# autonomousvision/LaRa

Hardware: AMD Instinct MI355X
Metric: novel-view frames/sec @512x512 (4-view in, 2DGS fwd+bwd) (higher is better)
Workload: dtype f32 raster + bf16-MFMA/f32-accumulate encoder (+ bf16-autocast coarse decoder MLP, as the reference's bf16-mixed)

## Files before the change

lara_amd/csrc/finedec.hip:

```cpp
#include "common.h"
#include "wave.h"
#include "../../include/lara_finedec.h"

namespace {

constexpr int FD = 80, NH = 8, CD = 8, NV = 4, HID = 64, SH = 12, TQ = NH * CD;

__device__ __forceinline__ int crow(const int tile, const int r, const int hf) { return tile * 32 + (r >> 2) * 8 + hf * 4 + (r & 3); }
__device__ __forceinline__ f32x16 mfma2(const float a, const float b, const f32x16 c) {
    return __builtin_amdgcn_mfma_f32_32x32x2f32(a, b, c, 0, 0, 0);
}
#define FD_FENCE(i, every) do { if (((i) % (every)) == (every) - 1) asm volatile("" ::: "memory"); } while (0)

__device__ __forceinline__ f32x16 zero16() {
    f32x16 z;
#pragma unroll
    for (int i = 0; i < 16; i++) z[i] = 0.f;
    return z;
}

constexpr int L_WQKT = 0;
constexpr int L_W1T = L_WQKT + FD * TQ;
constexpr int L_W2T = L_W1T + TQ * HID;
constexpr int L_B1 = L_W2T + HID * 32;
// ... 232 lines not shown
#pragma unroll
                for (int c = 0; c < 4; c++) {
                    dt[c] += dsc * pf[j][c];
                    dpf[j][c] += p[h][j] * du[mt][r0 + c] + dsc * t[mt][r0 + c];
                }
            }
#pragma unroll
            for (int c = 0; c < 4; c++) du[mt][r0 + c] = dt[c];
            asm volatile("" ::: "memory");
        }
        if (live) {
            store64(DT_g, pt, du);
#pragma unroll
            for (int j = 0; j < NV; j++)
#pragma unroll
                for (int c = 0; c < 4; c++) dpf_g[(int64_t)(j * CD + hf * 4 + c) * n + pt] = dpf[j][c];
        }
#pragma unroll
        for (int ft = 0; ft < 3; ft++) {
            f32x16 dx = zero16();
#pragma unroll
            for (int mt = 0; mt < 2; mt++)
#pragma unroll
                for (int r = 0; r < 16; r++) {
                    dx = mfma2(sw[L_WQK + crow(mt, r, hf) * 96 + ft * 32 + col], du[mt][r], dx);
                    FD_FENCE(r, 8);
                }
            if (live) {
#pragma unroll
                for (int q = 0; q < 4; q++) {
                    const int f0 = ft * 32 + q * 8 + hf * 4;
                    if (f0 < FD) *(float4 *)(dxn_g + pt * FD + f0) = make_float4(dx[4 * q], dx[4 * q + 1], dx[4 * q + 2], dx[4 * q + 3]);
                }
            }
        }
    }
}


__global__ void __launch_bounds__(256)
fine_ln_fwd_kernel(const int n, const float *__restrict__ x_g, const float *__restrict__ gamma, const float *__restrict__ beta,
                   const float eps, float *__restrict__ xn_g, float2 *__restrict__ stats) {
    __shared__ float sg[FD], sb[FD];
    if (threadIdx.x < FD) { sg[threadIdx.x] = gamma[threadIdx.x]; sb[threadIdx.x] = beta[threadIdx.x]; }
    __syncthreads();
    const int64_t i = (int64_t)blockIdx.x * 256 + threadIdx.x;
    if (i >= n) return;
    const float4 *x4 = (const float4 *)(x_g + i * FD);
    float4 v[FD / 4];
    float sum = 0.f;
#pragma unroll
    for (int k = 0; k < FD / 4; k++) { v[k] = x4[k]; sum += (v[k].x + v[k].y) + (v[k].z + v[k].w); }
    const float mean = sum * (1.0f / FD);
    float var = 0.f;
#pragma unroll
    for (int k = 0; k < FD / 4; k++) {
        const float a = v[k].x - mean, b = v[k].y - mean, c = v[k].z - mean, d = v[k].w - mean;
        var += (a * a + b * b) + (c * c + d * d);
    }
    const float rstd = 1.0f / sqrtf(var * (1.0f / FD) + eps);
    float4 *o4 = (float4 *)(xn_g + i * FD);
#pragma unroll
    for (int k = 0; k < FD / 4; k++) {
        float4 o;
        o.x = (v[k].x - mean) * rstd * sg[4 * k] + sb[4 * k];
        o.y = (v[k].y - mean) * rstd * sg[4 * k + 1] + sb[4 * k + 1];
        o.z = (v[k].z - mean) * rstd * sg[4 * k + 2] + sb[4 * k + 2];
        o.w = (v[k].w - mean) * rstd * sg[4 * k + 3] + sb[4 * k + 3];
        o4[k] = o;
    }
    stats[i] = make_float2(mean, rstd);
}

__device__ __forceinline__ float wave_sum_to_lane63(float x) {
    x += dpp_move<0xB1, 0xf>(x);
    x += dpp_move<0x4E, 0xf>(x);
    x += dpp_move<0x141, 0xf>(x);
    x += dpp_move<0x140, 0xf>(x);
    x += dpp_move<0x142, 0xa>(x);
    x += dpp_move<0x143, 0xc>(x);
    return x;
}

__global__ void __launch_bounds__(256)
fine_ln_bwd_kernel(const int n, const float *__restrict__ x_g, const float *__restrict__ gamma, const float2 *__restrict__ stats,
                   const float *__restrict__ dxn_g, float *__restrict__ dx_g, float *__restrict__ partials) {
    __shared__ float sg[FD];
    __shared__ float part[4][2 * FD];
    if (threadIdx.x < FD) sg[threadIdx.x] = gamma[threadIdx.x];
    __syncthreads();
    const int64_t i = (int64_t)blockIdx.x * 256 + threadIdx.x;
    const bool on = i < n;
    const int lane = threadIdx.x & 63, wave = threadIdx.x >> 6;
    float4 xh[FD / 4], g[FD / 4];
    float2 st = make_float2(0.f, 0.f);
    if (on) st = stats[i];
    float s1 = 0.f, s2 = 0.f;
#pragma unroll
    for (int k = 0; k < FD / 4; k++) {
        float4 xv = make_float4(0.f, 0.f, 0.f, 0.f), dv = xv;
        if (on) { xv = ((const float4 *)(x_g + i * FD))[k]; dv = ((const float4 *)(dxn_g + i * FD))[k]; }
        xh[k] = make_float4((xv.x - st.x) * st.y, (xv.y - st.x) * st.y, (xv.z - st.x) * st.y, (xv.w - st.x) * st.y);
        const float pg[4] = {dv.x * xh[k].x, dv.y * xh[k].y, dv.z * xh[k].z, dv.w * xh[k].w};
        const float pb[4] = {dv.x, dv.y, dv.z, dv.w};
#pragma unroll
        for (int q = 0; q < 4; q++) {
            const float a = wave_sum_to_lane63(pg[q]), b = wave_sum_to_lane63(pb[q]);
            if (lane == 63) { part[wave][4 * k + q] = a; part[wave][FD + 4 * k + q] = b; }
        }
        g[k] = make_float4(dv.x * sg[4 * k], dv.y * sg[4 * k + 1], dv.z * sg[4 * k + 2], dv.w * sg[4 * k + 3]);
        s1 += (g[k].x + g[k].y) + (g[k].z + g[k].w);
        s2 += (g[k].x * xh[k].x + g[k].y * xh[k].y) + (g[k].z * xh[k].z + g[k].w * xh[k].w);
    }
    if (on) {
        const float m1 = s1 * (1.0f / FD), m2 = s2 * (1.0f / FD);
        float4 *o4 = (float4 *)(dx_g + i * FD);
#pragma unroll
        for (int k = 0; k < FD / 4; k++)
            o4[k] = make_float4(st.y * (g[k].x - m1 - xh[k].x * m2), st.y * (g[k].y - m1 - xh[k].y * m2),
                                st.y * (g[k].z - m1 - xh[k].z * m2), st.y * (g[k].w - m1 - xh[k].w * m2));
    }
    __syncthreads();
    if (threadIdx.x < 2 * FD)
        partials[(size_t)blockIdx.x * 2 * FD + threadIdx.x] =
            ((part[0][threadIdx.x] + part[1][threadIdx.x]) + part[2][threadIdx.x]) + part[3][threadIdx.x];
}

constexpr int FW_SLAB = 512;
constexpr int FW_OUT = 64 * 80 + 64 * 64 + 64 + 12 * 64 + 12;
constexpr int FW_O_W1 = 64 * 80, FW_O_B1 = FW_O_W1 + 64 * 64, FW_O_W2 = FW_O_B1 + 64, FW_O_B2 = FW_O_W2 + 12 * 64;

template <int AV, int BV>
__device__ __forceinline__ void fw_store(float *__restrict__ out, const int ldo, const int i_rows, const int j_cols, const int lane,
                                         const f32x16 (&acc)[AV][BV]) {
    const int cB = lane & 31, kh = lane >> 5;
#pragma unroll
    for (int ea = 0; ea < AV; ea++)
#pragma unroll
        for (int eb = 0; eb < BV; eb++)
#pragma unroll
            for (int e = 0; e < 16; e++) {
                const int i = AV * ((e & 3) + 8 * (e >> 2) + 4 * kh) + ea, j = BV * cB + eb;
                if (i < i_rows && j < j_cols) out[(size_t)i * ldo + j] = acc[ea][eb][e];
            }
}

__global__ void __launch_bounds__(192)
fine_wgrad_kernel(const int n, const float *__restrict__ xn, const float *__restrict__ U, const float *__restrict__ HID_,
                  const float *__restrict__ DH, const float *__restrict__ DT, const float *__restrict__ d_sh,
                  float *__restrict__ part) {
    const int wave = threadIdx.x >> 6, lane = threadIdx.x & 63;
    const int row0 = blockIdx.x * FW_SLAB, rows = min(FW_SLAB, n - row0);
    float *out = part + (size_t)blockIdx.x * FW_OUT;
    const int kk = lane >> 5, c = lane & 31;
    constexpr int UN = 8;
    if (wave < 2) {
        f32x16 acc[2][2];
#pragma unroll
        for (int a = 0; a < 2; a++)
#pragma unroll
            for (int b = 0; b < 2; b++)
#pragma unroll
                for (int e = 0; e < 16; e++) acc[a][b][e] = 0.f;
        const bool b_ok = c < FD / 4;
        for (int r = 0; r < rows; r += 2 * UN) {
            float2 av[UN], bv[UN];
#pragma unroll
            for (int u = 0; u < UN; u++) {
                const int rr = r + 2 * u + kk;
                const bool in = rr < rows;
                av[u] = in ? *(const float2 *)(DT + (size_t)(row0 + rr) * 64 + 2 * c) : make_float2(0.f, 0.f);
                bv[u] = (in && b_ok) ? *(const float2 *)(xn + (size_t)(row0 + rr) * FD + 4 * c + 2 * wave) : make_float2(0.f, 0.f);
            }
#pragma unroll
            for (int u = 0; u < UN; u++) {
                acc[0][0] = mfma2(av[u].x, bv[u].x, acc[0][0]);
                acc[0][1] = mfma2(av[u].x, bv[u].y, acc[0][1]);
                acc[1][0] = mfma2(av[u].y, bv[u].x, acc[1][0]);
                acc[1][1] = mfma2(av[u].y, bv[u].y, acc[1][1]);
            }
        }
        const int kh = lane >> 5;
#pragma unroll
        for (int ea = 0; ea < 2; ea++)
#pragma unroll
            for (int eb = 0; eb < 2; eb++)
#pragma unroll
                for (int e = 0; e < 16; e++) {
                    const int i = 2 * ((e & 3) + 8 * (e >> 2) + 4 * kh) + ea, j = 4 * c + 2 * wave + eb;
                    if (j < FD) out[(size_t)i * FD + j] = acc[ea][eb][e];
                }
    } else {
        f32x16 acc1[2][2], acc2[1][2];
#pragma unroll
        for (int b = 0; b < 2; b++)
#pragma unroll
            for (int e = 0; e < 16; e++) { acc1[0][b][e] = 0.f; acc1[1][b][e] = 0.f; acc2[0][b][e] = 0.f; }
        float cs1x = 0.f, cs1y = 0.f, cs2 = 0.f;
        const bool s_ok = c < SH;
        for (int r = 0; r < rows; r += 2 * UN) {
            float2 dh[UN], uu[UN], hh[UN];
            float ds[UN];
#pragma unroll
// ... 133 lines not shown
```

lara_amd/csrc/pointfeat.hip:

```cpp
#include "common.h"
#include "../../include/lara_pointfeat.h"

namespace {

constexpr int PF_MAX_VIEWS = 8;

struct PfP {
    int n, V, h, w;
    const float *points, *w2cs, *ixts, *img_ref, *image, *acc, *depth;
    int vtot;
};

__device__ __forceinline__ size_t map_pixel(const PfP &p, const size_t i) {
    if (p.vtot == 0) return i;
    const size_t hw = (size_t)p.h * p.w, v = i / hw, pix = i - v * hw, y = pix / p.w, x = pix - y * p.w;
    return (y * p.vtot + v) * p.w + x;
}

struct Tap {
    int idx[4];
    float wgt[4];
    float wx, wy;
    bool in[4];
};
// ... 98 lines not shown
        const Proj pr = project(p, v, px, py, pz);
        const Tap t = taps(pr.x, pr.y, p.h, p.w);
        float val[4][8];
#pragma unroll
        for (int k = 0; k < 4; k++) {
            if (t.in[k]) chan8(packed, hw, v, t.idx[k], val[k]);
            else
#pragma unroll
                for (int c = 0; c < 8; c++) val[k][c] = 0.f;
        }
        float gx = 0.f, gy = 0.f, gz = 0.f, gc[8];
#pragma unroll
        for (int c = 0; c < 8; c++) {
            float g = g_out[((size_t)v * 8 + c) * p.n + i];
            if (c == 7) {
                const float s = t.wgt[0] * val[0][c] + t.wgt[1] * val[1][c] + t.wgt[2] * val[2][c] + t.wgt[3] * val[3][c];
                const float d = s - pr.z, sg = d > 0.f ? 1.f : d < 0.f ? -1.f : 0.f;
                gz -= sg * g;
                g *= sg;
            }
            gc[c] = g;
            gx += g * ((val[1][c] - val[0][c]) * (1.f - t.wy) + (val[3][c] - val[2][c]) * t.wy);
            gy += g * ((val[2][c] - val[0][c]) * (1.f - t.wx) + (val[3][c] - val[1][c]) * t.wx);
        }
        if (dpacked) {
#pragma unroll
            for (int k = 0; k < 4; k++) {
                s_off[wave][lane][k] = t.in[k] ? (int)(((size_t)v * hw + t.idx[k]) * 8) : -1;
                s_wgt[wave][lane][k] = t.wgt[k];
            }
#pragma unroll
            for (int c = 0; c < 8; c++) s_g[wave][lane][c] = gc[c];
        }
        const float inv = 1.0f / pr.z;
        const float dqx = gx * inv, dqy = gy * inv, dqz = gz - (gx * pr.x + gy * pr.y) * inv;
        const float *m = p.w2cs + v * 16, *k = p.ixts + v * 9;
        const float dcx = k[0] * dqx + k[3] * dqy + k[6] * dqz, dcy = k[1] * dqx + k[4] * dqy + k[7] * dqz,
                    dcz = k[2] * dqx + k[5] * dqy + k[8] * dqz;
        dpx = m[0] * dcx + m[4] * dcy + m[8] * dcz;
        dpy = m[1] * dcx + m[5] * dcy + m[9] * dcz;
        dpz = m[2] * dcx + m[6] * dcy + m[10] * dcz;
    }
    if (dpacked) {
        __builtin_amdgcn_wave_barrier();
        const int ch = lane & 7;
#pragma unroll 4
        for (int r = 0; r < 32; r++) {
            const int item = r * 8 + (lane >> 3), th = item >> 2, k = item & 3;
            const int off = s_off[wave][th][k];
            if (off >= 0 && ch >= 3) atomicAdd(dpacked + off + ch, s_wgt[wave][th][k] * s_g[wave][th][ch]);
        }
    }
#pragma unroll
    for (int o = 1; o < VP; o <<= 1) {
        dpx += __shfl_xor(dpx, o, 64); dpy += __shfl_xor(dpy, o, 64); dpz += __shfl_xor(dpz, o, 64);
    }
    if (active && v == 0) {
        d_points[3 * (size_t)i] = dpx; d_points[3 * (size_t)i + 1] = dpy; d_points[3 * (size_t)i + 2] = dpz;
    }
}

template <int VP>
int launch_fwd(const PfP &p, const float4 *packed, float *out, hipStream_t s) {
    const size_t threads = (size_t)p.n * VP;
    L2D_LAUNCH_IN_SCOPE(s, (point_feats_fwd_kernel<VP>), dim3((unsigned)((threads + 255) / 256)), dim3(256), 0, p, packed, out);
    return LARA2DGS_OK;
}
template <int VP>
int launch_bwd(const PfP &p, const float4 *packed, const float *g_out, float *d_points, float *dpacked, hipStream_t s) {
    const size_t threads = (size_t)p.n * VP;
    L2D_LAUNCH_IN_SCOPE(s, (point_feats_bwd_kernel<VP>), dim3((unsigned)((threads + 255) / 256)), dim3(256), 0, p, packed, g_out,
                        d_points, dpacked);
    return LARA2DGS_OK;
}
int launch_pack(const PfP &p, float4 *packed, hipStream_t s) {
    const size_t n = (size_t)p.V * p.h * p.w;
    L2D_LAUNCH_IN_SCOPE(s, pack_stack_kernel, dim3((unsigned)((n + 255) / 256)), dim3(256), 0, p, packed);
    return LARA2DGS_OK;
}

struct RowsP {
    const float *src[LARA_ROWS_MAX];
    float *dst[LARA_ROWS_MAX];
    int width[LARA_ROWS_MAX], first[LARA_ROWS_MAX + 1];
    const int64_t *idx;
    int n, count;
};
template <bool SCATTER>
__global__ void __launch_bounds__(256) take_rows_kernel(const RowsP p) {
    const int total = p.first[p.count];
    const int t = blockIdx.x * 256 + threadIdx.x;
    if (t >= p.n * total) return;
    const int r = t / total, c = t - r * total;
    int k = 0;
    while (k + 1 < p.count && c >= p.first[k + 1]) k++;
    const int w = p.width[k], cc = c - p.first[k];
    const size_t far = (size_t)p.idx[r] * w + cc, near = (size_t)r * w + cc;
    if (SCATTER) p.dst[k][far] = p.src[k][near];
    else p.dst[k][near] = p.src[k][far];
}

__global__ void __launch_bounds__(256) voxel_rows_fwd_kernel(const int n, const int c4, const long long *__restrict__ vox,
                                                            const float4 *__restrict__ x, float4 *__restrict__ out) {
    const long long t = (long long)blockIdx.x * 256 + threadIdx.x;
    if (t >= (long long)n * c4) return;
    const int r = (int)(t / c4), c = (int)(t - (long long)r * c4);
    out[t] = x[(size_t)vox[r] * c4 + c];
}
__global__ void __launch_bounds__(256) voxel_rows_bwd_kernel(const int n, const int c4, const long long *__restrict__ vox,
                                                            const float4 *__restrict__ g, float4 *__restrict__ dx) {
    const long long t = (long long)blockIdx.x * 256 + threadIdx.x;
    if (t >= (long long)n * c4) return;
    const int r = (int)(t / c4), c = (int)(t - (long long)r * c4);
    const long long v = vox[r];
    if (r > 0 && vox[r - 1] == v) return;
    float4 a = g[t];
    for (int q = r + 1; q < n && vox[q] == v; q++) {
        const float4 b = g[(size_t)q * c4 + c];
        a.x += b.x; a.y += b.y; a.z += b.z; a.w += b.w;
    }
    dx[(size_t)v * c4 + c] = a;
}

}

extern "C" {

int lara_voxel_rows(int32_t n, int32_t width, const int64_t *vox, const float *src, float *dst, int32_t backward, void *stream) {
    if (n < 0 || width <= 0 || (width & 3)) return LARA2DGS_E_INVALID;
    if (n == 0) return LARA2DGS_OK;
    if (!vox || !src || !dst) return LARA2DGS_E_INVALID;
    hipStream_t s = (hipStream_t)stream;
    const int c4 = width / 4;
    const unsigned blocks = (unsigned)(((long long)n * c4 + 255) / 256);
    {
        L2D_PROF(backward ? "voxel_rows_bwd" : "voxel_rows_fwd", s);
        if (backward) L2D_LAUNCH_IN_SCOPE(s, voxel_rows_bwd_kernel, dim3(blocks), dim3(256), 0, n, c4, (const long long *)vox, (const float4 *)src, (float4 *)dst);
        else L2D_LAUNCH_IN_SCOPE(s, voxel_rows_fwd_kernel, dim3(blocks), dim3(256), 0, n, c4, (const long long *)vox, (const float4 *)src, (float4 *)dst);
    }
    return LARA2DGS_OK;
}

int64_t lara_point_feats_workspace_bytes(int32_t V, int32_t h, int32_t w) {
    if (V <= 0 || V > PF_MAX_VIEWS || h <= 0 || w <= 0 || (int64_t)V * h * w * 8 >= (1ll << 31)) return LARA2DGS_E_INVALID;
    return (int64_t)V * h * w * 32 * 2;
}

int lara_point_feats_forward(int32_t n, int32_t V, int32_t h, int32_t w, const float *points, const float *w2cs,
                             const float *ixts, const float *img_ref, const float *image, const float *acc_map,
                             const float *depth, float *out, void *workspace, void *stream) {
    return lara_point_feats_forward_concat(n, V, 0, h, w, points, w2cs, ixts, img_ref, image, acc_map, depth, out, workspace, stream);
}

int lara_point_feats_forward_concat(int32_t n, int32_t V, int32_t row_views, int32_t h, int32_t w, const float *points,
                                    const float *w2cs, const float *ixts, const float *img_ref, const float *image,
                                    const float *acc_map, const float *depth, float *out, void *workspace, void *stream) {
    if (row_views < 0 || (row_views > 0 && row_views < V)) return LARA2DGS_E_INVALID;
    if (n < 0 || V <= 0 || V > PF_MAX_VIEWS || h <= 0 || w <= 0 || (int64_t)V * h * w * 8 >= (1ll << 31)) return LARA2DGS_E_INVALID;
    if (n == 0) return LARA2DGS_OK;
    if (!points || !w2cs || !ixts || !img_ref || !image || !acc_map || !depth || !out || !workspace) return LARA2DGS_E_INVALID;
    hipStream_t s = (hipStream_t)stream;
    const PfP p{n, V, h, w, points, w2cs, ixts, img_ref, image, acc_map, depth, row_views};
    float4 *packed = (float4 *)workspace;
    {
        L2D_PROF("point_feats_pack", s);
        L2D_TRY(launch_pack(p, packed, s));
    }
    {
        L2D_PROF("point_feats_fwd", s);
        if (V == 1) L2D_TRY(launch_fwd<1>(p, packed, out, s));
        else if (V == 2) L2D_TRY(launch_fwd<2>(p, packed, out, s));
        else if (V <= 4) L2D_TRY(launch_fwd<4>(p, packed, out, s));
        else L2D_TRY(launch_fwd<8>(p, packed, out, s));
    }
    return LARA2DGS_OK;
}

int lara_point_feats_backward(int32_t n, int32_t V, int32_t h, int32_t w, const float *points, const float *w2cs,
                              const float *ixts, const float *img_ref, const float *image, const float *acc_map,
                              const float *depth, const float *g_out, float *d_points, float *d_image,
                              float *d_acc_map, float *d_depth, void *workspace, void *stream) {
    return lara_point_feats_backward_concat(n, V, 0, h, w, points, w2cs, ixts, img_ref, image, acc_map, depth, g_out, d_points,
                                            d_image, d_acc_map, d_depth, workspace, stream);
}

int lara_point_feats_backward_concat(int32_t n, int32_t V, int32_t row_views, int32_t h, int32_t w, const float *points,
                                     const float *w2cs, const float *ixts, const float *img_ref, const float *image,
                                     const float *acc_map, const float *depth, const float *g_out, float *d_points,
                                     float *d_image, float *d_acc_map, float *d_depth, void *workspace, void *stream) {
    if (row_views < 0 || (row_views > 0 && row_views < V)) return LARA2DGS_E_INVALID;
    if (n < 0 || V <= 0 || V > PF_MAX_VIEWS || h <= 0 || w <= 0 || (int64_t)V * h * w * 8 >= (1ll << 31)) return LARA2DGS_E_INVALID;
    if (n == 0) return LARA2DGS_OK;
    if (!points || !w2cs || !ixts || !img_ref || !image || !acc_map || !depth || !g_out || !d_points || !workspace)
        return LARA2DGS_E_INVALID;
    hipStream_t s = (hipStream_t)stream;
    const PfP p{n, V, h, w, points, w2cs, ixts, img_ref, image, acc_map, depth, row_views};
    const size_t npix = (size_t)V * h * w;
    float4 *packed = (float4 *)workspace;
    const bool maps = d_image || d_acc_map || d_depth;
    float *dpacked = maps ? (float *)workspace + npix * 8 : nullptr;
    {
        L2D_PROF("point_feats_pack", s);
        L2D_TRY(launch_pack(p, packed, s));
        if (maps) L2D_HIP(hipMemsetAsync(dpacked, 0, npix * 32, s));
    }
    {
        L2D_PROF("point_feats_bwd", s);
        if (V == 1) L2D_TRY(launch_bwd<1>(p, packed, g_out, d_points, dpacked, s));
        else if (V == 2) L2D_TRY(launch_bwd<2>(p, packed, g_out, d_points, dpacked, s));
        else if (V <= 4) L2D_TRY(launch_bwd<4>(p, packed, g_out, d_points, dpacked, s));
        else L2D_TRY(launch_bwd<8>(p, packed, g_out, d_points, dpacked, s));
        if (maps)
            L2D_LAUNCH_IN_SCOPE(s, unpack_grad_kernel, dim3((unsigned)((npix + 255) / 256)), dim3(256), 0, p, (const float4 *)dpacked, npix,
                                d_image, d_acc_map, d_depth);
    }
    return LARA2DGS_OK;
}


int lara_take_rows(int32_t n, const int64_t *idx, int32_t count, const lara_rows_item *items, int32_t scatter, void *stream) {
    if (n < 0 || count < 0 || count > LARA_ROWS_MAX) return LARA2DGS_E_INVALID;
    if (n == 0 || count == 0) return LARA2DGS_OK;
    if (!idx || !items) return LARA2DGS_E_INVALID;
    RowsP p{};
    p.n = n; p.count = count; p.idx = idx;
    int total = 0;
    for (int k = 0; k < count; k++) {
        if (!items[k].src || !items[k].dst || items[k].width <= 0) return LARA2DGS_E_INVALID;
        p.src[k] = items[k].src; p.dst[k] = items[k].dst; p.width[k] = items[k].width; p.first[k] = total;
        total += items[k].width;
    }
    p.first[count] = total;
    if ((int64_t)n * total >= (1ll << 31)) return LARA2DGS_E_INVALID;
    hipStream_t s = (hipStream_t)stream;
    const unsigned blocks = (unsigned)(((int64_t)n * total + 255) / 256);
    {
        L2D_PROF(scatter ? "take_rows_bwd" : "take_rows_fwd", s);
        if (scatter) L2D_LAUNCH_IN_SCOPE(s, take_rows_kernel<true>, dim3(blocks), dim3(256), 0, p);
        else L2D_LAUNCH_IN_SCOPE(s, take_rows_kernel<false>, dim3(blocks), dim3(256), 0, p);
    }
    return LARA2DGS_OK;
}

}
```

lara_amd/csrc/preprocess.hip:

```cpp
#include "common.h"
#include "tilebox.h"

static_assert(TILE == 16, "tilebox.h's l2d_tight_rect cuts to 16-pixel tiles");

namespace {

__device__ __constant__ float kSH_C2[5] = {1.0925484305920792f, -1.0925484305920792f,
                                           0.31539156525252005f, -1.0925484305920792f,
                                           0.5462742152960396f};
__device__ __constant__ float kSH_C3[7] = {-0.5900435899266435f, 2.890611442640554f,
                                           -0.4570457994644658f, 0.3731763325901154f,
                                           -0.4570457994644658f, 1.445305721320277f,
                                           -0.5900435899266435f};
#define SH_C0 0.28209479177387814f
#define SH_C1 0.4886025119029199f

struct Pm43 { float m[4][3]; };

__device__ __forceinline__ Pm43 build_Pm(const ViewDev &v) {
    Pm43 r;
    const float hw = (float)v.W / 2.0f, hh = (float)v.H / 2.0f;
    const float cw = (float)(v.W - 1) / 2.0f, ch = (float)(v.H - 1) / 2.0f;
#pragma unroll
    for (int a = 0; a < 4; a++) {
// ... 239 lines not shown
    if (threadIdx.x == 255) block_tot[block] = woff + incl;
    if (idx < v.P) {
        const float depth = tt ? view_depth : 0.f;
        rect_out[idx] = make_uint4((uint32_t)r.x | ((uint32_t)r.y << 16), (uint32_t)r.z | ((uint32_t)r.w << 16),
                                   __float_as_uint(depth), woff + incl - tt);
    }
    for (int y = r.y; y < r.w; y++)
        for (int x = r.x; x < r.z; x++) {
            if (use_lds) atomicAdd(&hist[y * v.gx + x], 1u);
            else __hip_atomic_fetch_add(&tile_count[(y * v.gx + x) * L2D_SLICES + slice], 1u, __ATOMIC_RELAXED, __HIP_MEMORY_SCOPE_AGENT);
        }
    if (use_lds) {
        __syncthreads();
        for (int t = threadIdx.x; t < v.tiles; t += blockDim.x) {
            const uint32_t c = hist[t];
            if (c) __hip_atomic_fetch_add(&tile_count[t * L2D_SLICES + slice], c, __ATOMIC_RELAXED, __HIP_MEMORY_SCOPE_AGENT);
        }
    }
}

struct PreViews {
    int n;
    const float *bg[L2D_MAX_VIEWS], *viewmatrix[L2D_MAX_VIEWS], *projmatrix[L2D_MAX_VIEWS], *campos[L2D_MAX_VIEWS];
    float4 *geom[L2D_MAX_VIEWS], *cullbox[L2D_MAX_VIEWS];
    uint4 *rect[L2D_MAX_VIEWS];
    uint32_t *tile_count[L2D_MAX_VIEWS], *block_tot[L2D_MAX_VIEWS];
    int32_t *radii[L2D_MAX_VIEWS];
};

template <int DEG>
__global__ void __launch_bounds__(256)
preprocess_fwd_views_kernel(ViewDev v, PreViews pv, const float *__restrict__ means3D, const float *__restrict__ shs,
                            const float *__restrict__ colors_precomp, const float *__restrict__ opacities,
                            const float2 *__restrict__ scales, const float4 *__restrict__ rotations,
                            const float *__restrict__ transmat_precomp, const int use_lds) {
    extern __shared__ __attribute__((aligned(16))) uint32_t hist[];
    __shared__ uint32_t wsum[4];
    const int view = (int)(blockIdx.x % (unsigned)pv.n), block = (int)(blockIdx.x / (unsigned)pv.n);
    v.bg = pv.bg[view]; v.viewmatrix = pv.viewmatrix[view]; v.projmatrix = pv.projmatrix[view]; v.campos = pv.campos[view];
    preprocess_fwd_block<DEG>(v, block, means3D, shs, colors_precomp, opacities, scales, rotations, transmat_precomp,
                              pv.geom[view], pv.cullbox[view], pv.rect[view], pv.tile_count[view], pv.block_tot[view],
                              pv.radii[view], use_lds, hist, wsum);
}

__global__ void __launch_bounds__(256)
mark_visible_kernel(int P, const float *__restrict__ means3D, const float *__restrict__ viewmatrix,
                    uint8_t *__restrict__ present) {
    const int idx = blockIdx.x * blockDim.x + threadIdx.x;
    if (idx >= P) return;
    const float p[3] = {means3D[3 * idx], means3D[3 * idx + 1], means3D[3 * idx + 2]};
    float pv[3];
    point4x3(viewmatrix, p, pv);
    present[idx] = pv[2] > 0.2f;
}

template <int DEG>
struct SurfelGrad {
    static constexpr int NSH = (DEG + 1) * (DEG + 1) * 3;
    float dmean[3], m2out[2], dopac, dscale[2], drot[4], dT[9], dcol[3], dsh[NSH];
    __device__ __forceinline__ void zero() {
#pragma unroll
        for (int k = 0; k < 3; k++) { dmean[k] = 0.f; dcol[k] = 0.f; }
        m2out[0] = m2out[1] = dopac = dscale[0] = dscale[1] = 0.f;
#pragma unroll
        for (int k = 0; k < 4; k++) drot[k] = 0.f;
#pragma unroll
        for (int k = 0; k < 9; k++) dT[k] = 0.f;
#pragma unroll
        for (int k = 0; k < NSH; k++) dsh[k] = 0.f;
    }
    __device__ __forceinline__ void add(const SurfelGrad &o) {
#pragma unroll
        for (int k = 0; k < 3; k++) { dmean[k] += o.dmean[k]; dcol[k] += o.dcol[k]; }
        m2out[0] += o.m2out[0]; m2out[1] += o.m2out[1]; dopac += o.dopac; dscale[0] += o.dscale[0]; dscale[1] += o.dscale[1];
#pragma unroll
        for (int k = 0; k < 4; k++) drot[k] += o.drot[k];
#pragma unroll
        for (int k = 0; k < 9; k++) dT[k] += o.dT[k];
#pragma unroll
        for (int k = 0; k < NSH; k++) dsh[k] += o.dsh[k];
    }
};

template <int DEG>
__device__ __forceinline__ void
surfel_backward(const ViewDev &v, const int idx, const float *__restrict__ means3D, const float *__restrict__ shs,
                const float *__restrict__ colors_precomp, const float2 *__restrict__ scales,
                const float4 *__restrict__ rotations, const float *__restrict__ transmat_precomp,
                const int32_t *__restrict__ radii, const float4 *__restrict__ geom,
                const uint32_t *__restrict__ pair_base, const float4 *__restrict__ pair_grad,
                const uint8_t *__restrict__ pair_valid, SurfelGrad<DEG> &G) {
    G.zero();
    const bool visible = radii[idx] > 0;

    float gacc[GRAD_F];
#pragma unroll
    for (int k = 0; k < GRAD_F; k++) gacc[k] = 0.f;
    if (visible) {
        const uint32_t q0 = pair_base[idx], q1 = pair_base[idx + 1];
        for (uint32_t q = q0; q < q1; q++) {
            if (!pair_valid[q]) continue;
            const float4 *row = pair_grad + (size_t)q * (GRAD_F / 4);
#pragma unroll
            for (int k = 0; k < GRAD_F / 4; k++) {
                const float4 w4 = row[k];
                gacc[4 * k] += w4.x; gacc[4 * k + 1] += w4.y; gacc[4 * k + 2] += w4.z; gacc[4 * k + 3] += w4.w;
            }
        }
    }
    G.dopac = gacc[14];

    float dmean[3] = {0.f, 0.f, 0.f};
    float2 dscale = make_float2(0.f, 0.f);
    float4 drot = make_float4(0.f, 0.f, 0.f, 0.f);
    float dT[9];
#pragma unroll
    for (int k = 0; k < 9; k++) dT[k] = gacc[k];
    float m2out[3] = {0.f, 0.f, 0.f};

    if (visible) {
        const float4 *g = geom + (size_t)idx * 5;
        const float4 g0 = g[0], g1 = g[1], g2 = g[2], g4 = g[4];
        const float T0[3] = {g0.x, g0.y, g0.z};
        const float T1[3] = {g0.w, g1.x, g1.y};
        const float T3[3] = {g1.z, g1.w, g2.x};
        const float m2x = gacc[9], m2y = gacc[10];
        if (m2x != 0.0f || m2y != 0.0f) {
            const float t[3] = {9.0f, 9.0f, -1.0f};
            const float d = t[0] * T3[0] * T3[0] + t[1] * T3[1] * T3[1] + t[2] * T3[2] * T3[2];
            const float f[3] = {t[0] * (1.0f / d), t[1] * (1.0f / d), t[2] * (1.0f / d)};
            float dL_dT3[3], dL_df[3];
#pragma unroll
            for (int k = 0; k < 3; k++) {
                dT[0 + k] += m2x * f[k] * T3[k];
                dT[3 + k] += m2y * f[k] * T3[k];
                dL_dT3[k] = m2x * f[k] * T0[k] + m2y * f[k] * T1[k];
                dL_df[k] = m2x * T0[k] * T3[k] + m2y * T1[k] * T3[k];
            }
            const float dL_dd = (dL_df[0] * f[0] + dL_df[1] * f[1] + dL_df[2] * f[2]) * (-1.0f / d);
#pragma unroll
            for (int k = 0; k < 3; k++) {
                dL_dT3[k] += dL_dd * (t[k] * T3[k] * 2.0f);
                dT[6 + k] += dL_dT3[k];
            }
        }
        const float p[3] = {means3D[3 * idx], means3D[3 * idx + 1], means3D[3 * idx + 2]};
        if (transmat_precomp == nullptr) {
            const Pm43 Pm = build_Pm(v);
            float Tm[3][3], normal[3], R[3][3], qn[4];
            const float2 sc = scales[idx];
            compute_transmat(v, Pm, p, sc, rotations[idx], Tm, normal, R, qn);
            float dM[3][3];
#pragma unroll
            for (int i = 0; i < 3; i++)
#pragma unroll
                for (int a = 0; a < 3; a++)
                    dM[i][a] = dT[0 + i] * Pm.m[a][0] + dT[3 + i] * Pm.m[a][1] + dT[6 + i] * Pm.m[a][2];
            const float dn[3] = {gacc[11], gacc[12], gacc[13]};
            float dtn[3];
            vec4x3T(v.viewmatrix, dn, dtn);
            float p_view[3];
            point4x3(v.viewmatrix, p, p_view);
            const float cosv = -(p_view[0] * normal[0] + p_view[1] * normal[1] + p_view[2] * normal[2]);
            const float mult = cosv > 0.0f ? 1.0f : -1.0f;
            dtn[0] *= mult; dtn[1] *= mult; dtn[2] *= mult;
            const float sx = v.scale_modifier * sc.x, sy = v.scale_modifier * sc.y;
            float V[3][3];
#pragma unroll
            for (int r = 0; r < 3; r++) { V[r][0] = dM[0][r] * sx; V[r][1] = dM[1][r] * sy; V[r][2] = dtn[r]; }
            dscale.x = v.scale_modifier * (dM[0][0] * R[0][0] + dM[0][1] * R[1][0] + dM[0][2] * R[2][0]);
            dscale.y = v.scale_modifier * (dM[1][0] * R[0][1] + dM[1][1] * R[1][1] + dM[1][2] * R[2][1]);
            const float w = qn[0], x = qn[1], y = qn[2], z = qn[3];
            drot.x = 2.f * (x * (V[2][1] - V[1][2]) + y * (V[0][2] - V[2][0]) + z * (V[1][0] - V[0][1]));
            drot.y = 2.f * (-2.f * x * (V[1][1] + V[2][2]) + y * (V[1][0] + V[0][1]) + z * (V[2][0] + V[0][2]) + w * (V[2][1] - V[1][2]));
            drot.z = 2.f * (x * (V[1][0] + V[0][1]) - 2.f * y * (V[0][0] + V[2][2]) + z * (V[2][1] + V[1][2]) + w * (V[0][2] - V[2][0]));
            drot.w = 2.f * (x * (V[2][0] + V[0][2]) + y * (V[2][1] + V[1][2]) - 2.f * z * (V[0][0] + V[1][1]) + w * (V[1][0] - V[0][1]));
            dmean[0] = dM[2][0]; dmean[1] = dM[2][1]; dmean[2] = dM[2][2];
        }

        if (colors_precomp == nullptr) {
            const float *sh = shs + (size_t)idx * v.M * 3;
            float *dsh = G.dsh;
            const float dir_o[3] = {p[0] - v.campos[0], p[1] - v.campos[1], p[2] - v.campos[2]};
            const float len = sqrtf(dir_o[0] * dir_o[0] + dir_o[1] * dir_o[1] + dir_o[2] * dir_o[2]);
            const float x = dir_o[0] / len, y = dir_o[1] / len, z = dir_o[2] / len;
            const uint32_t clamp_bits = __float_as_uint(g4.w);
            float ddir[3] = {0.f, 0.f, 0.f};
#pragma unroll
            for (int ch = 0; ch < 3; ch++) {
                const float gg = gacc[15 + ch] * ((clamp_bits >> ch) & 1u ? 0.0f : 1.0f);
                float dx = 0.f, dy = 0.f, dz = 0.f;
                dsh[0 * 3 + ch] = SH_C0 * gg;
                if (DEG > 0) {
                    const float s1 = sh[1 * 3 + ch], s2 = sh[2 * 3 + ch], s3 = sh[3 * 3 + ch];
                    dsh[1 * 3 + ch] = -SH_C1 * y * gg;
                    dsh[2 * 3 + ch] = SH_C1 * z * gg;
                    dsh[3 * 3 + ch] = -SH_C1 * x * gg;
                    dx = -SH_C1 * s3; dy = -SH_C1 * s1; dz = SH_C1 * s2;
                    if (DEG > 1) {
                        const float xx = x * x, yy = y * y, zz = z * z, xy = x * y, yz = y * z, xz = x * z;
                        const float s4 = sh[4 * 3 + ch], s5 = sh[5 * 3 + ch], s6 = sh[6 * 3 + ch],
                                    s7 = sh[7 * 3 + ch], s8 = sh[8 * 3 + ch];
                        dsh[4 * 3 + ch] = kSH_C2[0] * xy * gg;
                        dsh[5 * 3 + ch] = kSH_C2[1] * yz * gg;
                        dsh[6 * 3 + ch] = kSH_C2[2] * (2.f * zz - xx - yy) * gg;
// ... 24 lines not shown
                            dz += kSH_C3[1] * s10 * xy + kSH_C3[2] * s11 * 4.f * 2.f * yz +
                                  kSH_C3[3] * s12 * 3.f * (2.f * zz - xx - yy) +
                                  kSH_C3[4] * s13 * 4.f * 2.f * xz + kSH_C3[5] * s14 * (xx - yy);
                        }
                    }
                }
                ddir[0] += dx * gg; ddir[1] += dy * gg; ddir[2] += dz * gg;
            }
            const float sum2 = dir_o[0] * dir_o[0] + dir_o[1] * dir_o[1] + dir_o[2] * dir_o[2];
            const float invsum32 = 1.0f / sqrtf(sum2 * sum2 * sum2);
            dmean[0] += ((sum2 - dir_o[0] * dir_o[0]) * ddir[0] - dir_o[1] * dir_o[0] * ddir[1] - dir_o[2] * dir_o[0] * ddir[2]) * invsum32;
            dmean[1] += (-dir_o[0] * dir_o[1] * ddir[0] + (sum2 - dir_o[1] * dir_o[1]) * ddir[1] - dir_o[2] * dir_o[1] * ddir[2]) * invsum32;
            dmean[2] += (-dir_o[0] * dir_o[2] * ddir[0] - dir_o[1] * dir_o[2] * ddir[1] + (sum2 - dir_o[2] * dir_o[2]) * ddir[2]) * invsum32;
        }
        const float depth = g2.x;
        m2out[0] = gacc[2] * depth * 0.5f * (float)v.W;
        m2out[1] = gacc[5] * depth * 0.5f * (float)v.H;
    }

#pragma unroll
    for (int k = 0; k < 3; k++) { G.dmean[k] = dmean[k]; G.dcol[k] = gacc[15 + k]; }
    G.m2out[0] = m2out[0]; G.m2out[1] = m2out[1];
    G.dscale[0] = dscale.x; G.dscale[1] = dscale.y;
    G.drot[0] = drot.x; G.drot[1] = drot.y; G.drot[2] = drot.z; G.drot[3] = drot.w;
#pragma unroll
    for (int k = 0; k < 9; k++) G.dT[k] = visible ? dT[k] : 0.f;
}

template <int DEG>
__device__ __forceinline__ void
write_surfel_grad(const ViewDev &v, const int idx, const SurfelGrad<DEG> &G, const bool has_sh, const bool has_col,
                  const bool has_tm, float *__restrict__ dL_dmeans3D, float *__restrict__ dL_dmeans2D,
                  float *__restrict__ dL_dshs, float *__restrict__ dL_dcolors, float *__restrict__ dL_dopacities,
                  float2 *__restrict__ dL_dscales, float4 *__restrict__ dL_drots, float *__restrict__ dL_dtransmat) {
    dL_dopacities[idx] = G.dopac;
    dL_dmeans3D[3 * idx + 0] = G.dmean[0];
    dL_dmeans3D[3 * idx + 1] = G.dmean[1];
    dL_dmeans3D[3 * idx + 2] = G.dmean[2];
    dL_dmeans2D[3 * idx + 0] = G.m2out[0];
    dL_dmeans2D[3 * idx + 1] = G.m2out[1];
    dL_dmeans2D[3 * idx + 2] = 0.f;
    if (!has_tm) {
        dL_dscales[idx] = make_float2(G.dscale[0], G.dscale[1]);
        dL_drots[idx] = make_float4(G.drot[0], G.drot[1], G.drot[2], G.drot[3]);
    } else {
#pragma unroll
        for (int k = 0; k < 9; k++) dL_dtransmat[9 * (size_t)idx + k] = G.dT[k];
    }
    if (has_sh) {
        float *dsh = dL_dshs + (size_t)idx * v.M * 3;
#pragma unroll
        for (int k = 0; k < SurfelGrad<DEG>::NSH; k++) dsh[k] = G.dsh[k];
        for (int k = SurfelGrad<DEG>::NSH; k < v.M * 3; k++) dsh[k] = 0.f;
    }
    if (has_col) {
#pragma unroll
        for (int ch = 0; ch < 3; ch++) dL_dcolors[3 * (size_t)idx + ch] = G.dcol[ch];
    }
}

struct BwdViews {
    int n;
    const float *viewmatrix[L2D_MAX_VIEWS], *projmatrix[L2D_MAX_VIEWS], *campos[L2D_MAX_VIEWS];
    const int32_t *radii[L2D_MAX_VIEWS];
    const float4 *geom[L2D_MAX_VIEWS], *pair_grad[L2D_MAX_VIEWS];
    const uint32_t *pair_base[L2D_MAX_VIEWS];
    const uint8_t *pair_valid[L2D_MAX_VIEWS];
};

template <int DEG, bool FOLD>
__global__ void __launch_bounds__(256)
preprocess_bwd_views_kernel(ViewDev v, BwdViews bv, const int accumulate, const float *__restrict__ means3D,
                            const float *__restrict__ shs, const float *__restrict__ colors_precomp,
                            const float2 *__restrict__ scales, const float4 *__restrict__ rotations,
                            const float *__restrict__ transmat_precomp, float *__restrict__ dL_dmeans3D,
                            float *__restrict__ dL_dmeans2D, float *__restrict__ dL_dshs, float *__restrict__ dL_dcolors,
                            float *__restrict__ dL_dopacities, float2 *__restrict__ dL_dscales,
                            float4 *__restrict__ dL_drots, float *__restrict__ dL_dtransmat) {
    const int idx = blockIdx.x * blockDim.x + threadIdx.x;
    if (idx >= v.P) return;
    const bool has_sh = colors_precomp == nullptr, has_col = !has_sh, has_tm = transmat_precomp != nullptr;
    SurfelGrad<DEG> A;
    if (!FOLD) {
        surfel_backward<DEG>(v, idx, means3D, shs, colors_precomp, scales, rotations, transmat_precomp, bv.radii[0],
                             bv.geom[0], bv.pair_base[0], bv.pair_grad[0], bv.pair_valid[0], A);
        write_surfel_grad<DEG>(v, idx, A, has_sh, has_col, has_tm, dL_dmeans3D, dL_dmeans2D, dL_dshs, dL_dcolors,
                               dL_dopacities, dL_dscales, dL_drots, dL_dtransmat);
        return;
    }
    if (accumulate) {
        A.zero();
        A.dopac = dL_dopacities[idx];
        for (int k = 0; k < 3; k++) A.dmean[k] = dL_dmeans3D[3 * idx + k];
        A.m2out[0] = dL_dmeans2D[3 * idx]; A.m2out[1] = dL_dmeans2D[3 * idx + 1];
        if (!has_tm) {
            const float2 a = dL_dscales[idx]; const float4 b = dL_drots[idx];
            A.dscale[0] = a.x; A.dscale[1] = a.y; A.drot[0] = b.x; A.drot[1] = b.y; A.drot[2] = b.z; A.drot[3] = b.w;
        } else {
            for (int k = 0; k < 9; k++) A.dT[k] = dL_dtransmat[9 * (size_t)idx + k];
        }
        if (has_sh) for (int k = 0; k < SurfelGrad<DEG>::NSH; k++) A.dsh[k] = dL_dshs[(size_t)idx * v.M * 3 + k];
        if (has_col) for (int k = 0; k < 3; k++) A.dcol[k] = dL_dcolors[3 * (size_t)idx + k];
    }
#pragma unroll 1
    for (int view = 0; view < bv.n; view++) {
        v.viewmatrix = bv.viewmatrix[view]; v.projmatrix = bv.projmatrix[view]; v.campos = bv.campos[view];
        SurfelGrad<DEG> G;
        surfel_backward<DEG>(v, idx, means3D, shs, colors_precomp, scales, rotations, transmat_precomp, bv.radii[view],
                             bv.geom[view], bv.pair_base[view], bv.pair_grad[view], bv.pair_valid[view], G);
        if (view == 0 && !accumulate) A = G;
        else A.add(G);
    }
    write_surfel_grad<DEG>(v, idx, A, has_sh, has_col, has_tm, dL_dmeans3D, dL_dmeans2D, dL_dshs, dL_dcolors, dL_dopacities,
                           dL_dscales, dL_drots, dL_dtransmat);
}

}

int launch_preprocess_fwd_views(const ViewDev &v, int n, const ViewDev *views, bool multi, const float *means3D, const float *shs,
                                const float *colors_precomp, const float *opacities, const float *scales,
                                const float *rotations, const float *transmat_precomp, const StateView *st,
                                const ScratchView *sc, int32_t *const *radii, hipStream_t s) {
    if (v.P == 0 || n <= 0) return LARA2DGS_OK;
    if (n > L2D_MAX_VIEWS) return LARA2DGS_E_INVALID;
    PreViews pv{};
    pv.n = n;
    for (int i = 0; i < n; i++) {
        pv.bg[i] = views[i].bg; pv.viewmatrix[i] = views[i].viewmatrix; pv.projmatrix[i] = views[i].projmatrix;
        pv.campos[i] = views[i].campos;
        pv.geom[i] = st[i].geom; pv.cullbox[i] = st[i].cullbox; pv.rect[i] = sc[i].rect;
        pv.tile_count[i] = sc[i].tile_count; pv.block_tot[i] = sc[i].block_tot; pv.radii[i] = radii[i];
    }
    const dim3 grid((unsigned)((v.P + 255) / 256) * (unsigned)n), block(256);
    const int use_lds = v.tiles <= L2D_LDS_HIST_TILES;
    const size_t lds_bytes = use_lds ? (size_t)v.tiles * 4 : 0;
#define L2D_PREV(DEG)                                                                                     \
    L2D_LAUNCH_IN_SCOPE(s, preprocess_fwd_views_kernel<DEG>, grid, block, lds_bytes, v, pv, means3D, shs, \
                        colors_precomp, opacities, (const float2 *)scales, (const float4 *)rotations,     \
                        transmat_precomp, use_lds)
    {
        L2D_PROF(multi ? "preprocess_fwd_views" : "preprocess_fwd", s);
        switch (colors_precomp ? 0 : v.deg) {
        case 0: L2D_PREV(0); break;
        case 1: L2D_PREV(1); break;
        case 2: L2D_PREV(2); break;
        default: L2D_PREV(3); break;
        }
    }
#undef L2D_PREV
    return LARA2DGS_OK;
}

int launch_mark_visible(int P, const float *means3D, const float *viewmatrix, uint8_t *present,
                        hipStream_t s) {
    if (P == 0) return LARA2DGS_OK;
    L2D_LAUNCH_IN_SCOPE(s, mark_visible_kernel, dim3((P + 255) / 256), dim3(256), 0, P, means3D,
                        viewmatrix, present);
    return LARA2DGS_OK;
}

int launch_preprocess_bwd_views(const ViewDev &v, int n, const ViewDev *views, bool multi, int accumulate, const float *means3D,
                                const float *shs, const float *colors_precomp, const float *scales, const float *rotations,
                                const float *transmat_precomp, const int32_t *const *radii, const StateView *st,
                                const ScratchView *sc, float *dL_dmeans3D, float *dL_dmeans2D, float *dL_dshs,
                                float *dL_dcolors, float *dL_dopacities, float *dL_dscales, float *dL_drotations,
                                float *dL_dtransmat, hipStream_t s) {
    if (v.P == 0 || n <= 0) return LARA2DGS_OK;
    if (n > L2D_MAX_VIEWS) return LARA2DGS_E_INVALID;
    BwdViews bv{};
    bv.n = n;
    for (int i = 0; i < n; i++) {
        bv.viewmatrix[i] = views[i].viewmatrix; bv.projmatrix[i] = views[i].projmatrix; bv.campos[i] = views[i].campos;
        bv.radii[i] = radii[i]; bv.geom[i] = st[i].geom; bv.pair_base[i] = st[i].pair_base;
        bv.pair_grad[i] = (const float4 *)sc[i].pair_grad; bv.pair_valid[i] = (const uint8_t *)sc[i].pair_valid;
    }
    const dim3 grid((v.P + 255) / 256), block(256);
    const bool fold = n > 1 || accumulate;
#define L2D_PREBV(DEG)                                                                                                      \
    L2D_LAUNCH_IN_SCOPE(s, (fold ? preprocess_bwd_views_kernel<DEG, true> : preprocess_bwd_views_kernel<DEG, false>), grid, \
                        block, 0, v, bv, accumulate, means3D, shs, colors_precomp, (const float2 *)scales,                  \
                        (const float4 *)rotations, transmat_precomp, dL_dmeans3D, dL_dmeans2D, dL_dshs, dL_dcolors,         \
                        dL_dopacities, (float2 *)dL_dscales, (float4 *)dL_drotations, dL_dtransmat)
    {
        L2D_PROF(multi ? "preprocess_bwd_views" : "preprocess_bwd", s);
        switch (colors_precomp ? 0 : v.deg) {
        case 0: L2D_PREBV(0); break;
        case 1: L2D_PREBV(1); break;
        case 2: L2D_PREBV(2); break;
        default: L2D_PREBV(3); break;
        }
    }
#undef L2D_PREBV
// ... 3 lines not shown
```

Baseline: 972.1.

## Coalesce LN backward via LDS tiles, per-row take_rows, prefetch surfel heads

Result: no change. 975.3, median of 6 (+0.3%).

```diff
diff --git a/lara_amd/csrc/finedec.hip b/lara_amd/csrc/finedec.hip
--- a/lara_amd/csrc/finedec.hip
+++ b/lara_amd/csrc/finedec.hip
@@ -338,43 +338,83 @@
     return x;
 }
 
+constexpr int LNB_K = 10;
+constexpr int LNB_PITCH = 4 * LNB_K + 4;
+static_assert((FD / 4) % LNB_K == 0, "whole chunks");
+
+__device__ __forceinline__ void lnb_load(const float *__restrict__ g, const int64_t row0, const int64_t n, const int ch, const int lane,
+                                         float4 (&t)[LNB_K]) {
+#pragma unroll
+    for (int j = 0; j < LNB_K; j++) {
+        const int f = j * 64 + lane, r = f / LNB_K, c = f - r * LNB_K;
+        t[j] = row0 + r < n ? *(const float4 *)(g + (row0 + r) * FD + 4 * (ch * LNB_K + c)) : make_float4(0.f, 0.f, 0.f, 0.f);
+    }
+}
+__device__ __forceinline__ void lnb_park(float *__restrict__ tile, const int lane, const float4 (&t)[LNB_K]) {
+#pragma unroll
+    for (int j = 0; j < LNB_K; j++) {
+        const int f = j * 64 + lane, r = f / LNB_K, c = f - r * LNB_K;
+        *(float4 *)(tile + r * LNB_PITCH + 4 * c) = t[j];
+    }
+}
+
 __global__ void __launch_bounds__(256)
 fine_ln_bwd_kernel(const int n, const float *__restrict__ x_g, const float *__restrict__ gamma, const float2 *__restrict__ stats,
                    const float *__restrict__ dxn_g, float *__restrict__ dx_g, float *__restrict__ partials) {
     __shared__ float sg[FD];
     __shared__ float part[4][2 * FD];
+    __shared__ __attribute__((aligned(16))) float tiles[4][2][64 * LNB_PITCH];
     if (threadIdx.x < FD) sg[threadIdx.x] = gamma[threadIdx.x];
-    __syncthreads();
-    const int64_t i = (int64_t)blockIdx.x * 256 + threadIdx.x;
+    const int lane = threadIdx.x & 63, wave = threadIdx.x >> 6;
+    const int64_t row0 = (int64_t)blockIdx.x * 256 + wave * 64, i = row0 + lane;
     const bool on = i < n;
-    const int lane = threadIdx.x & 63, wave = threadIdx.x >> 6;
+    float *tx = tiles[wave][0], *td = tiles[wave][1];
     float4 xh[FD / 4], g[FD / 4];
     float2 st = make_float2(0.f, 0.f);
     if (on) st = stats[i];
     float s1 = 0.f, s2 = 0.f;
-#pragma unroll
-    for (int k = 0; k < FD / 4; k++) {
-        float4 xv = make_float4(0.f, 0.f, 0.f, 0.f), dv = xv;
-        if (on) { xv = ((const float4 *)(x_g + i * FD))[k]; dv = ((const float4 *)(dxn_g + i * FD))[k]; }
-        xh[k] = make_float4((xv.x - st.x) * st.y, (xv.y - st.x) * st.y, (xv.z - st.x) * st.y, (xv.w - st.x) * st.y);
-        const float pg[4] = {dv.x * xh[k].x, dv.y * xh[k].y, dv.z * xh[k].z, dv.w * xh[k].w};
-        const float pb[4] = {dv.x, dv.y, dv.z, dv.w};
-#pragma unroll
-        for (int q = 0; q < 4; q++) {
-            const float a = wave_sum_to_lane63(pg[q]), b = wave_sum_to_lane63(pb[q]);
-            if (lane == 63) { part[wave][4 * k + q] = a; part[wave][FD + 4 * k + q] = b; }
-        }
-        g[k] = make_float4(dv.x * sg[4 * k], dv.y * sg[4 * k + 1], dv.z * sg[4 * k + 2], dv.w * sg[4 * k + 3]);
-        s1 += (g[k].x + g[k].y) + (g[k].z + g[k].w);
-        s2 += (g[k].x * xh[k].x + g[k].y * xh[k].y) + (g[k].z * xh[k].z + g[k].w * xh[k].w);
-    }
-    if (on) {
-        const float m1 = s1 * (1.0f / FD), m2 = s2 * (1.0f / FD);
-        float4 *o4 = (float4 *)(dx_g + i * FD);
-#pragma unroll
-        for (int k = 0; k < FD / 4; k++)
-            o4[k] = make_float4(st.y * (g[k].x - m1 - xh[k].x * m2), st.y * (g[k].y - m1 - xh[k].y * m2),
-                                st.y * (g[k].z - m1 - xh[k].z * m2), st.y * (g[k].w - m1 - xh[k].w * m2));
+    float4 lx[LNB_K], ld[LNB_K];
+    lnb_load(x_g, row0, n, 0, lane, lx); lnb_load(dxn_g, row0, n, 0, lane, ld);
+#pragma unroll
+    for (int ch = 0; ch < FD / 4 / LNB_K; ch++) {
+        lnb_park(tx, lane, lx); lnb_park(td, lane, ld);
+        if (ch + 1 < FD / 4 / LNB_K) { lnb_load(x_g, row0, n, ch + 1, lane, lx); lnb_load(dxn_g, row0, n, ch + 1, lane, ld); }
+        __syncthreads();
+#pragma unroll
+        for (int kk = 0; kk < LNB_K; kk++) {
+            const int k = ch * LNB_K + kk;
+            const float4 xv = *(const float4 *)(tx + lane * LNB_PITCH + 4 * kk), dv = *(const float4 *)(td + lane * LNB_PITCH + 4 * kk);
+            xh[k] = make_float4((xv.x - st.x) * st.y, (xv.y - st.x) * st.y, (xv.z - st.x) * st.y, (xv.w - st.x) * st.y);
+            const float pg[4] = {dv.x * xh[k].x, dv.y * xh[k].y, dv.z * xh[k].z, dv.w * xh[k].w};
+            const float pb[4] = {dv.x, dv.y, dv.z, dv.w};
+#pragma unroll
+            for (int q = 0; q < 4; q++) {
+                const float a = wave_sum_to_lane63(pg[q]), b = wave_sum_to_lane63(pb[q]);
+                if (lane == 63) { part[wave][4 * k + q] = a; part[wave][FD + 4 * k + q] = b; }
+            }
+            g[k] = make_float4(dv.x * sg[4 * k], dv.y * sg[4 * k + 1], dv.z * sg[4 * k + 2], dv.w * sg[4 * k + 3]);
+            s1 += (g[k].x + g[k].y) + (g[k].z + g[k].w);
+            s2 += (g[k].x * xh[k].x + g[k].y * xh[k].y) + (g[k].z * xh[k].z + g[k].w * xh[k].w);
+        }
+        __syncthreads();
+    }
+    const float m1 = s1 * (1.0f / FD), m2 = s2 * (1.0f / FD);
+#pragma unroll
+    for (int ch = 0; ch < FD / 4 / LNB_K; ch++) {
+        float *to = tiles[wave][ch & 1];
+#pragma unroll
+        for (int kk = 0; kk < LNB_K; kk++) {
+            const int k = ch * LNB_K + kk;
+            *(float4 *)(to + lane * LNB_PITCH + 4 * kk) =
+                make_float4(st.y * (g[k].x - m1 - xh[k].x * m2), st.y * (g[k].y - m1 - xh[k].y * m2),
+                            st.y * (g[k].z - m1 - xh[k].z * m2), st.y * (g[k].w - m1 - xh[k].w * m2));
+        }
+        __syncthreads();
+#pragma unroll
+        for (int j = 0; j < LNB_K; j++) {
+            const int f = j * 64 + lane, r = f / LNB_K, c = f - r * LNB_K;
+            if (row0 + r < n) *(float4 *)(dx_g + (row0 + r) * FD + 4 * (ch * LNB_K + c)) = *(const float4 *)(to + r * LNB_PITCH + 4 * c);
+        }
     }
     __syncthreads();
     if (threadIdx.x < 2 * FD)
diff --git a/lara_amd/csrc/pointfeat.hip b/lara_amd/csrc/pointfeat.hip
--- a/lara_amd/csrc/pointfeat.hip
+++ b/lara_amd/csrc/pointfeat.hip
@@ -204,22 +204,28 @@
 struct RowsP {
     const float *src[LARA_ROWS_MAX];
     float *dst[LARA_ROWS_MAX];
-    int width[LARA_ROWS_MAX], first[LARA_ROWS_MAX + 1];
+    int width[LARA_ROWS_MAX], vec[LARA_ROWS_MAX];
     const int64_t *idx;
     int n, count;
 };
+template <class V>
+__device__ __forceinline__ void copy_row(const float *__restrict__ s, float *__restrict__ d, const int w) {
+    constexpr int E = (int)(sizeof(V) / sizeof(float));
+    for (int c = 0; c < w; c += E) *(V *)(d + c) = *(const V *)(s + c);
+}
 template <bool SCATTER>
 __global__ void __launch_bounds__(256) take_rows_kernel(const RowsP p) {
-    const int total = p.first[p.count];
-    const int t = blockIdx.x * 256 + threadIdx.x;
-    if (t >= p.n * total) return;
-    const int r = t / total, c = t - r * total;
-    int k = 0;
-    while (k + 1 < p.count && c >= p.first[k + 1]) k++;
-    const int w = p.width[k], cc = c - p.first[k];
-    const size_t far = (size_t)p.idx[r] * w + cc, near = (size_t)r * w + cc;
-    if (SCATTER) p.dst[k][far] = p.src[k][near];
-    else p.dst[k][near] = p.src[k][far];
+    const int r = blockIdx.x * 256 + threadIdx.x;
+    if (r >= p.n) return;
+    const size_t far = (size_t)p.idx[r], from = SCATTER ? (size_t)r : far, to = SCATTER ? far : (size_t)r;
+    for (int k = 0; k < p.count; k++) {
+        const int w = p.width[k];
+        const float *s = p.src[k] + from * w;
+        float *d = p.dst[k] + to * w;
+        if (p.vec[k] == 4) copy_row<float4>(s, d, w);
+        else if (p.vec[k] == 2) copy_row<float2>(s, d, w);
+        else copy_row<float>(s, d, w);
+    }
 }
 
 __global__ void __launch_bounds__(256) voxel_rows_fwd_kernel(const int n, const int c4, const long long *__restrict__ vox,
@@ -349,13 +355,14 @@
     int total = 0;
     for (int k = 0; k < count; k++) {
         if (!items[k].src || !items[k].dst || items[k].width <= 0) return LARA2DGS_E_INVALID;
-        p.src[k] = items[k].src; p.dst[k] = items[k].dst; p.width[k] = items[k].width; p.first[k] = total;
+        p.src[k] = items[k].src; p.dst[k] = items[k].dst; p.width[k] = items[k].width;
+        const uintptr_t where = (uintptr_t)items[k].src | (uintptr_t)items[k].dst | ((uintptr_t)items[k].width * 4);
+        p.vec[k] = where % 16 == 0 ? 4 : where % 8 == 0 ? 2 : 1;
         total += items[k].width;
     }
-    p.first[count] = total;
     if ((int64_t)n * total >= (1ll << 31)) return LARA2DGS_E_INVALID;
     hipStream_t s = (hipStream_t)stream;
-    const unsigned blocks = (unsigned)(((int64_t)n * total + 255) / 256);
+    const unsigned blocks = (unsigned)((n + 255) / 256);
     {
         L2D_PROF(scatter ? "take_rows_bwd" : "take_rows_fwd", s);
         if (scatter) L2D_LAUNCH_IN_SCOPE(s, take_rows_kernel<true>, dim3(blocks), dim3(256), 0, p);
diff --git a/lara_amd/csrc/preprocess.hip b/lara_amd/csrc/preprocess.hip
--- a/lara_amd/csrc/preprocess.hip
+++ b/lara_amd/csrc/preprocess.hip
@@ -345,24 +345,47 @@
     }
 };
 
-template <int DEG>
+struct SurfelHead {
+    int32_t radius;
+    uint32_t q0, q1;
+};
+__device__ __forceinline__ SurfelHead load_head(const int32_t *__restrict__ radii, const uint32_t *__restrict__ pair_base, const int idx) {
+    SurfelHead h;
+    h.radius = radii[idx]; h.q0 = pair_base[idx]; h.q1 = pair_base[idx + 1];
+    return h;
+}
+__device__ __forceinline__ uint32_t first_valid(const SurfelHead &h, const uint8_t *__restrict__ pair_valid) {
+    return (h.radius > 0 && h.q0 < h.q1) ? pair_valid[h.q0] : 0u;
+}
+
+template <int DEG, bool AHEAD, class AfterRows>
 __device__ __forceinline__ void
 surfel_backward(const ViewDev &v, const int idx, const float *__restrict__ means3D, const float *__restrict__ shs,
                 const float *__restrict__ colors_precomp, const float2 *__restrict__ scales,
                 const float4 *__restrict__ rotations, const float *__restrict__ transmat_precomp,
                 const int32_t *__restrict__ radii, const float4 *__restrict__ geom,
                 const uint32_t *__restrict__ pair_base, const float4 *__restrict__ pair_grad,
-                const uint8_t *__restrict__ pair_valid, SurfelGrad<DEG> &G) {
+                const uint8_t *__restrict__ pair_valid, SurfelGrad<DEG> &G, const SurfelHead h, uint32_t ok,
+                AfterRows &&after_rows) {
     G.zero();
-    const bool visible = radii[idx] > 0;
+    const bool visible = AHEAD ? h.radius > 0 : radii[idx] > 0;
+    float4 g0, g1, g2, g4;
+    if (AHEAD && visible) {
+        const float4 *g = geom + (size_t)idx * 5;
+        g0 = g[0]; g1 = g[1]; g2 = g[2]; g4 = g[4];
+    }
 
     float gacc[GRAD_F];
 #pragma unroll
     for (int k = 0; k < GRAD_F; k++) gacc[k] = 0.f;
     if (visible) {
-        const uint32_t q0 = pair_base[idx], q1 = pair_base[idx + 1];
+        const uint32_t q0 = AHEAD ? h.q0 : pair_base[idx], q1 = AHEAD ? h.q1 : pair_base[idx + 1];
         for (uint32_t q = q0; q < q1; q++) {
-            if (!pair_valid[q]) continue;
+            if (AHEAD) {
+                const uint32_t ok_now = ok;
+                ok = q + 1 < q1 ? pair_valid[q + 1] : 0u;
+                if (!ok_now) continue;
+            } else if (!pair_valid[q]) continue;
             const float4 *row = pair_grad + (size_t)q * (GRAD_F / 4);
 #pragma unroll
             for (int k = 0; k < GRAD_F / 4; k++) {
@@ -371,6 +394,7 @@
             }
         }
     }
+    after_rows();
     G.dopac = gacc[14];
 
     float dmean[3] = {0.f, 0.f, 0.f};
@@ -382,8 +406,10 @@
     float m2out[3] = {0.f, 0.f, 0.f};
 
     if (visible) {
-        const float4 *g = geom + (size_t)idx * 5;
-        const float4 g0 = g[0], g1 = g[1], g2 = g[2], g4 = g[4];
+        if (!AHEAD) {
+            const float4 *g = geom + (size_t)idx * 5;
+            g0 = g[0]; g1 = g[1]; g2 = g[2]; g4 = g[4];
+        }
         const float T0[3] = {g0.x, g0.y, g0.z};
         const float T1[3] = {g0.w, g1.x, g1.y};
         const float T3[3] = {g1.z, g1.w, g2.x};
@@ -574,8 +600,8 @@
     const bool has_sh = colors_precomp == nullptr, has_col = !has_sh, has_tm = transmat_precomp != nullptr;
     SurfelGrad<DEG> A;
     if (!FOLD) {
-        surfel_backward<DEG>(v, idx, means3D, shs, colors_precomp, scales, rotations, transmat_precomp, bv.radii[0],
-                             bv.geom[0], bv.pair_base[0], bv.pair_grad[0], bv.pair_valid[0], A);
+        surfel_backward<DEG, false>(v, idx, means3D, shs, colors_precomp, scales, rotations, transmat_precomp, bv.radii[0],
+                                    bv.geom[0], bv.pair_base[0], bv.pair_grad[0], bv.pair_valid[0], A, SurfelHead{}, 0u, [] {});
         write_surfel_grad<DEG>(v, idx, A, has_sh, has_col, has_tm, dL_dmeans3D, dL_dmeans2D, dL_dshs, dL_dcolors,
                                dL_dopacities, dL_dscales, dL_drots, dL_dtransmat);
         return;
@@ -594,12 +620,28 @@
         if (has_sh) for (int k = 0; k < SurfelGrad<DEG>::NSH; k++) A.dsh[k] = dL_dshs[(size_t)idx * v.M * 3 + k];
         if (has_col) for (int k = 0; k < 3; k++) A.dcol[k] = dL_dcolors[3 * (size_t)idx + k];
     }
+    constexpr bool AHEAD = DEG < 3;
+    SurfelHead h{};
+    uint32_t ok0 = 0;
+    if (AHEAD) { h = load_head(bv.radii[0], bv.pair_base[0], idx); ok0 = first_valid(h, bv.pair_valid[0]); }
 #pragma unroll 1
     for (int view = 0; view < bv.n; view++) {
         v.viewmatrix = bv.viewmatrix[view]; v.projmatrix = bv.projmatrix[view]; v.campos = bv.campos[view];
         SurfelGrad<DEG> G;
-        surfel_backward<DEG>(v, idx, means3D, shs, colors_precomp, scales, rotations, transmat_precomp, bv.radii[view],
-                             bv.geom[view], bv.pair_base[view], bv.pair_grad[view], bv.pair_valid[view], G);
+        if (AHEAD) {
+            const int nxt = view + 1 < bv.n ? view + 1 : view;
+            const SurfelHead nh = load_head(bv.radii[nxt], bv.pair_base[nxt], idx);
+            const uint8_t *valid_nxt = bv.pair_valid[nxt];
+            uint32_t nok0 = 0;
+            surfel_backward<DEG, true>(v, idx, means3D, shs, colors_precomp, scales, rotations, transmat_precomp, bv.radii[view],
+                                       bv.geom[view], bv.pair_base[view], bv.pair_grad[view], bv.pair_valid[view], G, h, ok0,
+                                       [&] { nok0 = first_valid(nh, valid_nxt); });
+            h = nh; ok0 = nok0;
+        } else {
+            surfel_backward<DEG, false>(v, idx, means3D, shs, colors_precomp, scales, rotations, transmat_precomp, bv.radii[view],
+                                        bv.geom[view], bv.pair_base[view], bv.pair_grad[view], bv.pair_valid[view], G, SurfelHead{},
+                                        0u, [] {});
+        }
         if (view == 0 && !accumulate) A = G;
         else A.add(G);
     }
```
